# ewrfcas/LeftRefill

Hardware: AMD Instinct MI355X
Metric: 512x1024 stitched images/sec @ 50 DDIM steps, cfg=2.5; per-UNet-step ms (higher is better)
Workload: dtype f16; 1 GPU; configs[1]: 1-ref inpainting, 512x1024 canvas (latent 64x128), B=4 per GPU (UNet batch 8 under CFG), 50 DDIM steps, cfg=2.5, eta=1.0, fp16; global_batch=4, per_gpu_batch=4, ddim_steps=50, parallelism=dp1 (sample-sharded, no data-path collective), ranks=1

## Files before the change

include/leftrefill_hip.h:

```cpp
#ifndef LEFTREFILL_HIP_H
#define LEFTREFILL_HIP_H

#include <stdint.h>

#ifdef __cplusplus
extern "C" {
#endif

#define LR_E_ARG (-1)
#define LR_E_ALIGN (-2)
#define LR_E_UNSUPPORTED (-3)

typedef void* lr_stream_t;
typedef uint16_t lr_half;
#define LR_DTYPE_F16 0
#define LR_DTYPE_BF16 1
#define LR_PIPE_DEFAULT 0
#define LR_PIPE_W8_DEEP 4
#define LR_PIPE_HALO 8
#define LR_UP_PHASE 3

int lr_abi_version(void);

int lr_nchw_f32_to_nhwc_f16(const float* x1, int C1, const float* x2, int C2, lr_half* y, int Cpad, int N, int H,
// ... 53 lines not shown
} lr_gemm_args;
int lr_gemm_gn_group_chunks(const lr_gemm_args* args);
int lr_gemm_gn_rows(const lr_gemm_args* args);
int lr_gemm_plan(const lr_gemm_args* args, int32_t* plan);
int lr_gemm_stats_parts(const lr_gemm_args* args);
int64_t lr_gemm_workspace_bytes(const lr_gemm_args* args);
int lr_gemm_conv_f16(const lr_gemm_args* args, lr_stream_t s);
int lr_gemm_splitk_timeouts(void);

int lr_attention_f16(const lr_half* q, int ldq, const lr_half* k, int ldk, const lr_half* v, int ldv, lr_half* o,
                     int ldo, int B, int heads, int Nq, int Nkv, float scale, lr_stream_t s);

int lr_attention_causal_f16(const lr_half* q, int ldq, const lr_half* k, int ldk, const lr_half* v, int ldv, lr_half* o,
                            int ldo, int B, int heads, int N, float scale, lr_stream_t s);
int lr_attention_vt_f16(const lr_half* q, int ldq, const lr_half* k, int ldk, const lr_half* vt, int ld_vt, lr_half* o,
                        int ldo, int B, int heads, int Nq, int Nkv, float scale, lr_stream_t s);
int lr_transpose_v_f16(const lr_half* v, int ldv, lr_half* vt, int ld_vt, int B, int heads, int Nkv, lr_stream_t s);

typedef struct lr_xattn_args {
  const lr_half* x; lr_half* out;
  const lr_half* wq; const float* bq;
  const lr_half* k; int32_t ldk;
  const lr_half* vt;
  const lr_half* wo; const float* bo;
  float* stats_out;
  int32_t M, HW, C, heads, Lc;
  float ln_eps, scale;
  const lr_half* pre_a; const lr_half* pre_w; const float* pre_b;
} lr_xattn_args;
int lr_xattn_block_f16(const lr_xattn_args* args, lr_stream_t s);
int lr_xattn_pack_vt_f16(const lr_half* v, int ldv, lr_half* vt, int B, int heads, int Lc, lr_stream_t s);

typedef struct lr_stin_args {
  const lr_half* x; const lr_half* wp; const float* bp; const lr_half* wqkv; const float* bqkv;
  lr_half* x1; lr_half* qkv;
  int32_t M, C, NQ, ld_qkv;
  float ln_eps;
  const float* gn_part; const float* gn_gamma; const float* gn_beta;
  int32_t gn_chunks, gn_hw;
  float gn_eps;
} lr_stin_args;
int lr_stin_block_f16(const lr_stin_args* args, lr_stream_t s);

typedef struct lr_rowlin_args {
  const lr_half* x; const lr_half* w; const float* bias; lr_half* out;
  int32_t M, C, N, ld_out, geglu;
  float ln_eps;
  int32_t ln;
  const float* gn_part; const float* gn_gamma; const float* gn_beta;
  int32_t gn_chunks, gn_hw;
  float gn_eps;
} lr_rowlin_args;
int lr_rowlin_f16(const lr_rowlin_args* args, lr_stream_t s);

typedef struct lr_ffn_args {
  const lr_half* x; lr_half* out;
  const lr_half* w1; const float* b1;
  const lr_half* w2; const float* b2;
  float* stats_out;
  int32_t M, C, H;
  float ln_eps;
  const lr_half* post_w; const float* post_b; const lr_half* post_resid; float* gn_stats_out;
  float* gn_group_out; int32_t gn_hw;
} lr_ffn_args;
int lr_ffn_block_f16(const lr_ffn_args* args, lr_stream_t s);

int lr_softmax_rows_f16(const lr_half* s, lr_half* p, int M, int N, float scale, lr_stream_t st);

int lr_mv_gather(const lr_half* x, lr_half* seq, int b, int v, int s, int C, lr_stream_t st);
typedef struct lr_row_copy_job {
  const void* src; int64_t src_pitch, src_off;
  void* dst; int64_t dst_pitch, dst_off;
  int32_t row_bytes, n_rows;
  const int32_t* src_idx; const int32_t* dst_idx;
} lr_row_copy_job;
int lr_row_copy(const lr_row_copy_job* jobs, int n_jobs, lr_stream_t s);
int lr_mv_scatter(const lr_half* seq, lr_half* x, int b, int v, int s, int C, lr_stream_t st);

int lr_ddim_cfg_step(const float* x, const void* eps, int eps_is_f32, const float* noise, float* x_prev,
                     float* pred_x0, int64_t numel, float cfg_scale, float a_t, float a_prev, float sigma_t,
                     float sqrt_one_minus_at, lr_stream_t s);

int lr_plms_cfg_step(const float* x, const void* eps, int eps_is_f32, const float* const* hist, int n_hist, const float* weights,
                     float divisor, float* e_out, float* x_prev, float* pred_x0, int64_t numel, float cfg_scale, float a_t,
                     float a_prev, float sqrt_one_minus_at, lr_stream_t s);

int lr_dpmpp_cfg_step(const float* x, const void* eps, int eps_is_f32, const float* x0_prev, float* x0_out, float* x_next,
                      int64_t numel, float cfg_scale, float sigma_s, float alpha_s, float ratio, float c, float c_half,
                      float inv_r0, lr_stream_t s);

int lr_ddim_inv_cfg_step(const float* x, const void* eps, int eps_is_f32, float* x_next, int64_t numel, float cfg_scale,
                         float c1, float c2, lr_stream_t s);

int lr_ddim_cfg3_step(const float* x, const void* eps, int eps_is_f32, const float* noise, float* x_prev, float* pred_x0,
                      int64_t numel, float cfg_scale, float cond_weight, float one_minus_cond_weight, float a_t, float a_prev,
                      float sigma_t, float sqrt_one_minus_at, lr_stream_t s);

int lr_ddpm_step(const float* x, const void* eps, int eps_is_f32, const float* noise, const float* known_x0,
                 const float* known_noise, const float* mask, int64_t mask_chw, int64_t mask_hw, int clip_denoised, float* x_prev,
                 float* x0_out, int64_t numel, float sqrt_recip_ac, float sqrt_recipm1_ac, float coef1, float coef2, float sigma,
                 float sqrt_ac, float sqrt_one_minus_ac, lr_stream_t s);

#define LR_Q_SAMPLE_MAX_B 32
int lr_ddim_q_sample(const float* x0, const float* noise, float* out, int B, int64_t per_sample, const float* sa,
                     const float* s1ma, lr_stream_t s);

// ... 280 lines not shown
```

leftrefill_amd/_lib.py:

```python
import ctypes
import os

HERE = os.path.dirname(os.path.abspath(__file__))
LIB_PATH = os.environ.get("LEFTREFILL_LIB_PATH") or os.path.join(HERE, "lib", "libleftrefill_hip.so")
ABI_VERSION = 30

c_void_p, c_int, c_float, c_int64 = ctypes.c_void_p, ctypes.c_int, ctypes.c_float, ctypes.c_int64


class GemmArgs(ctypes.Structure):
    _fields_ = [
        ("p1", c_void_p), ("C1", ctypes.c_int32),
        ("p2", c_void_p), ("C2", ctypes.c_int32),
        ("B", ctypes.c_int32), ("H", ctypes.c_int32), ("W", ctypes.c_int32),
        ("Hs", ctypes.c_int32), ("Ws", ctypes.c_int32),
        ("taps", ctypes.c_int32), ("stride", ctypes.c_int32), ("up", ctypes.c_int32),
        ("asym", ctypes.c_int32),
        ("wt", c_void_p), ("N", ctypes.c_int32),
        ("bias", c_void_p),
        ("rowvec", c_void_p), ("ld_rowvec", ctypes.c_int32),
        ("resid", c_void_p), ("ld_resid", ctypes.c_int32),
        ("out", c_void_p), ("ld_out", ctypes.c_int32),
        ("geglu", ctypes.c_int32),
        ("tile_n", ctypes.c_int32),
# ... 147 lines not shown
                                    c_float, c_void_p],
    "lr_attention_causal_bwd_f16": [ctypes.POINTER(AttnBwdArgs), c_void_p],
    "lr_gelu_fwd_f16": [c_void_p, c_void_p, c_int64, c_void_p],
    "lr_gelu_bwd_f16": [c_void_p, c_void_p, c_void_p, c_int64, c_void_p],
    "lr_transpose_v_f16": [c_void_p, c_int, c_void_p, c_int, c_int, c_int, c_int, c_void_p],
    "lr_xattn_block_f16": [ctypes.POINTER(XattnArgs), c_void_p],
    "lr_xattn_pack_vt_f16": [c_void_p, c_int, c_void_p, c_int, c_int, c_int, c_void_p],
    "lr_ffn_block_f16": [ctypes.POINTER(FfnArgs), c_void_p],
    "lr_stin_block_f16": [ctypes.POINTER(StinArgs), c_void_p],
    "lr_rowlin_f16": [ctypes.POINTER(RowlinArgs), c_void_p],
    "lr_mv_gather": [c_void_p, c_void_p, c_int, c_int, c_int, c_int, c_void_p],
    "lr_row_copy": [c_void_p, c_int, c_void_p],
    "lr_gemm_splitk_timeouts": [],
    "lr_mv_scatter": [c_void_p, c_void_p, c_int, c_int, c_int, c_int, c_void_p],
    "lr_ddim_cfg_step": [c_void_p, c_void_p, c_int, c_void_p, c_void_p, c_void_p, c_int64, c_float, c_float, c_float,
                         c_float, c_float, c_void_p],
    "lr_timestep_embedding_f32": [c_void_p, c_int, c_int, c_void_p, c_void_p],
    "lr_plms_cfg_step": [c_void_p, c_void_p, c_int, c_void_p, c_int, c_void_p, c_float, c_void_p, c_void_p, c_void_p, c_int64,
                         c_float, c_float, c_float, c_float, c_void_p],
    "lr_dpmpp_cfg_step": [c_void_p, c_void_p, c_int, c_void_p, c_void_p, c_void_p, c_int64, c_float, c_float, c_float, c_float,
                          c_float, c_float, c_float, c_void_p],
    "lr_ddim_inv_cfg_step": [c_void_p, c_void_p, c_int, c_void_p, c_int64, c_float, c_float, c_float, c_void_p],
    "lr_ddim_cfg3_step": [c_void_p, c_void_p, c_int, c_void_p, c_void_p, c_void_p, c_int64, c_float, c_float, c_float, c_float,
                          c_float, c_float, c_float, c_void_p],
    "lr_ddpm_step": [c_void_p, c_void_p, c_int, c_void_p, c_void_p, c_void_p, c_void_p, c_int64, c_int64, c_int, c_void_p, c_void_p,
                     c_int64, c_float, c_float, c_float, c_float, c_float, c_float, c_float, c_void_p],
    "lr_ddim_q_sample": [c_void_p, c_void_p, c_void_p, c_int, c_int64, c_void_p, c_void_p, c_void_p],
    "lr_eval_metrics": [c_void_p, c_int, c_void_p, c_void_p, c_int, c_int, c_int, c_int, c_int, c_int, c_void_p, c_void_p, c_void_p,
                        c_void_p],
    "lr_amp_adamw_step": [c_void_p, c_int, c_void_p, c_int, c_void_p, c_void_p, c_int, c_float, c_float, c_int,
                          ctypes.POINTER(c_int), c_void_p],
    "lr_lpips_workspace_bytes": [c_int, c_int, c_int, c_int],
    "lr_lpips_alex": [ctypes.POINTER(LpipsArgs), c_void_p],
    "lr_batch_prep": [c_void_p, c_int64, c_void_p, c_void_p, c_int, c_int, c_int, c_int, c_void_p, c_void_p, c_void_p, c_void_p],
    "lr_nvs_prep": [c_void_p, c_int64, c_void_p, c_void_p, c_int, c_int, c_void_p, c_void_p, c_void_p, c_void_p],
    "lr_pil_resize": [c_void_p, c_int64, c_void_p, c_void_p, c_int64, c_void_p, c_int64, c_void_p, c_int64, c_void_p, c_void_p, c_int,
                      c_void_p],
    "lr_refill_canvas": [c_void_p, c_void_p, c_void_p, c_int, c_int, c_int, c_int, c_int, c_int, c_void_p, c_void_p, c_void_p, c_void_p],
    "lr_image_grid": [ctypes.POINTER(GridSource), c_int, c_int, c_int, c_int, c_int, c_void_p, c_int, c_void_p],
    "lr_token_drift": [c_void_p, c_void_p, c_int, c_int, c_void_p, c_void_p],
    "lr_attention_probe_f16": [c_void_p, c_int, c_void_p, c_int, c_void_p, c_int, c_int, c_void_p, c_int, c_int, c_int, c_int, c_float,
                               c_float, c_float, c_void_p],
    "lr_lora_down_f16": [c_void_p, c_int, c_void_p, c_int, c_void_p, c_int, c_int, c_int, c_int, c_float, c_void_p],
    "lr_lora_up_f16": [c_void_p, c_int, c_void_p, c_int, c_void_p, c_int, c_int, c_int, c_int, c_int, c_void_p],
    "lr_lora_wgrad_workspace_bytes": [c_int, c_int, c_int],
    "lr_lora_wgrad_f16": [c_void_p, c_int, c_void_p, c_int, c_void_p, c_int, c_int, c_int, c_int, c_float, c_void_p, c_int64, c_void_p],
    "lr_lora_merge_f32": [c_void_p, c_void_p, c_void_p, c_void_p, c_int, c_int, c_int, c_float, c_void_p],
    "lr_lora_down_drop_f16": [c_void_p, c_int, c_void_p, c_int, c_void_p, c_int, c_int, c_int, c_int, c_float, ctypes.POINTER(LoraDrop),
                              c_void_p],
    "lr_lora_up_drop_f16": [c_void_p, c_int, c_void_p, c_int, c_void_p, c_int, c_int, c_int, c_int, c_int, ctypes.POINTER(LoraDrop),
                            c_void_p],
    "lr_lora_wgrad_drop_f16": [c_void_p, c_int, c_void_p, c_int, c_void_p, c_int, c_int, c_int, c_int, c_float, c_void_p, c_int64,
                               ctypes.POINTER(LoraDrop), c_void_p],
}
INT64_RETURNS = ("lr_gemm_workspace_bytes", "lr_lpips_workspace_bytes", "lr_lora_wgrad_workspace_bytes")

BF16_TWINS = ["lr_groupnorm_stats", "lr_groupnorm_apply", "lr_groupnorm_apply_n", "lr_layernorm", "lr_layernorm_bwd",
              "lr_groupnorm_bwd", "lr_layernorm_bwd_res", "lr_groupnorm_bwd_res", "lr_nchw_f32_to_nhwc_f16", "lr_nhwc_f16_to_nchw", "lr_timestep_embedding", "lr_linear_small_m",
              "lr_mv_gather", "lr_mv_scatter", "lr_ddim_cfg_step", "lr_timestep_embedding_f32", "lr_plms_cfg_step",
              "lr_dpmpp_cfg_step", "lr_ddim_inv_cfg_step", "lr_ddim_cfg3_step", "lr_ddpm_step", "lr_geglu_fwd", "lr_geglu_bwd", "lr_sumpool2x2",
              "lr_mv_gather_bwd", "lr_mv_scatter_bwd", "lr_attention_f16", "lr_attention_causal_f16", "lr_attention_lse_f16",
              "lr_attention_vt_f16", "lr_transpose_v_f16", "lr_attention_bwd_f16", "lr_xattn_block_f16",
              "lr_xattn_pack_vt_f16", "lr_ffn_block_f16", "lr_stin_block_f16", "lr_rowlin_f16", "lr_gn_conv_out_f16",
              "lr_attention_causal_lse_f16", "lr_attention_causal_bwd_f16", "lr_gelu_fwd_f16", "lr_gelu_bwd_f16",
              "lr_attention_probe_f16", "lr_lora_down_f16", "lr_lora_up_f16", "lr_lora_wgrad_f16",
              "lr_lora_down_drop_f16", "lr_lora_up_drop_f16", "lr_lora_wgrad_drop_f16"]


def twin(name):
    return (name[:-4] if name.endswith("_f16") else name) + "_bf16"


for _n in BF16_TWINS:
    SIGNATURES[twin(_n)] = SIGNATURES[_n]

_FOLD_SIG = [c_void_p, c_int, c_int, c_int, c_int, c_void_p, c_void_p, c_float, c_void_p, c_void_p, c_int, c_void_p, c_void_p, c_void_p]
DEV_SIGNATURES = {"lr_dev_set": [ctypes.c_char_p, c_int], "lr_dev_unset": [ctypes.c_char_p],
                  "lr_gn_fold_weights_f16": _FOLD_SIG, "lr_gn_fold_weights_bf16": _FOLD_SIG}

_lib = None


def fn(lib, name, dtype):
    import torch
    if dtype == torch.bfloat16:
        return getattr(lib, twin(name))
    assert dtype == torch.float16, dtype
    return getattr(lib, name)


def load():
    global _lib
    if _lib is not None:
        return _lib
    import torch
    if not os.path.exists(LIB_PATH):
        raise RuntimeError(
            f"{LIB_PATH} not found: build it with `python -m leftrefill_amd.build` (hipcc --offload-arch=gfx950). "
            "leftrefill_amd has no fallback path.")
    lib = ctypes.CDLL(LIB_PATH)
    for name, argtypes in SIGNATURES.items():
        fn = getattr(lib, name)
        fn.argtypes = argtypes
        fn.restype = c_int64 if name in INT64_RETURNS else c_int
    v = lib.lr_abi_version()
    if v != ABI_VERSION:
# ... 32 lines not shown
```

leftrefill_amd/csrc/rowlin.hip:

```cpp
#include "chain_common.h"

#define RL_ROWS 128
#define RL_THREADS 512
#define RL_SLOT 40960
#ifndef RL_DMA_AUX
#define RL_DMA_AUX 0
#endif
#ifndef RL_DEPTH
#define RL_DEPTH 1
#endif
#ifndef RL_W4_DEFAULT
#define RL_W4_DEFAULT 0
#endif
#define RL_MAX_SLICE 2560

struct RowlinParams {
  const void* x; const void* w; const float* bias; void* out;
  int M, N, ld_out, ny, np;
  float eps;
  const float* gn_part; const float* gn_gamma; const float* gn_beta; int gn_chunks, gn_hw; float gn_eps;
};

template <typename T, int C, bool GEGLU, bool LN, bool GN = false>
__global__ __launch_bounds__(RL_THREADS) void rowlin_kernel(const RowlinParams P) {
#if defined(__HIP_DEVICE_COMPILE__)
  constexpr int KL = C / 64;
  constexpr int NKS = C / 320;
  constexpr int RS = C == 320 ? 2 : 1;
  constexpr int UPR = GEGLU ? 1 : 2;
  constexpr int NU = RS * UPR;
  constexpr int S = NU;
  extern __shared__ __attribute__((aligned(16))) char smem[];
  float* par = reinterpret_cast<float*>(smem + 3 * RL_SLOT);

  const int t = threadIdx.x, lane = t & 63;
  const int w = __builtin_amdgcn_readfirstlane(t >> 6);
  const int fr = lane & 15, fq = lane >> 4;
  const int odd = fq & 1, ch8 = (fq >> 1) * 8;
  const int rb = blockIdx.x / P.ny, y = blockIdx.x - rb * P.ny;
  const int m_w0 = rb * (RL_ROWS * RS) + w * 16 * RS;
  const int np = P.np;
  const int g_base = y * np;
  const int j0 = rb % np;

  vec8<T> xf[RS][KL][2];
#pragma unroll
  for (int rs = 0; rs < RS; ++rs) {
    const T* xrow = reinterpret_cast<const T*>(P.x) + (size_t)(m_w0 + 16 * rs + fr) * C + 8 * fq;
#pragma unroll
    for (int t5 = 0; t5 < KL; ++t5)
#pragma unroll
      for (int u = 0; u < 2; ++u) xf[rs][t5][u] = *reinterpret_cast<const vec8<T>*>(xrow + 64 * t5 + 32 * u);
  }
  for (int i = t; i < np * 16; i += RL_THREADS)
    *reinterpret_cast<f32x4*>(par + 4 * i) = *reinterpret_cast<const f32x4*>(P.bias + (size_t)g_base * 64 + 4 * i);

  const __amdgpu_buffer_rsrc_t rsW = uniform_rsrc(P.w, (size_t)P.N * C * 2);
  const unsigned OOB = 0x80000000u;
  const int lrow = w * 8 + (lane >> 3);
  const int lchunk = (lane & 7) ^ ((lrow >> 1) & 7);
  const unsigned vrow = (unsigned)((lrow * C + lchunk * 8) * 2);
  auto issue = [&](int slot, int g, int kh, int i, bool live) __attribute__((always_inline)) {
    __builtin_amdgcn_raw_ptr_buffer_load_lds(rsW, (lptr_t)(smem + slot * RL_SLOT + (i * 64 + w * 8) * 128), 16, live ? vrow : OOB,
                                             (g * 64 * C + 320 * kh + i * 64) * 2, 0, RL_DMA_AUX);
  };
  auto piece_of = [&](int j) -> int { const int q = j0 + j; return g_base + (q < np ? q : q - np); };
  {
    const int g0 = piece_of(0);
#pragma unroll
    for (int i = 0; i < 5; ++i) issue(0, g0, 0, i, true);
#pragma unroll
    for (int i = 0; i < 5; ++i) {
      if constexpr (NKS == 1) issue(1, np > 1 ? piece_of(1) : g0, 0, i, np > 1); else issue(1, g0, 1, i, true);
    }
  }

  if constexpr (GN) {
    float* tabA = par + RL_MAX_SLICE;
    float* tabB = tabA + C;
    xa_gn_tables(P.gn_part, P.gn_chunks, (rb * (RL_ROWS * RS)) / P.gn_hw, P.gn_hw, C, P.gn_gamma, P.gn_beta, P.gn_eps, tabA, tabB, tabB + C, t, RL_THREADS);
#pragma unroll
    for (int rs = 0; rs < RS; ++rs)
#pragma unroll
      for (int t5 = 0; t5 < KL; ++t5)
#pragma unroll
        for (int u = 0; u < 2; ++u) {
          const int c0 = 64 * t5 + 32 * u + 8 * fq;
          const f32x4 a0 = *reinterpret_cast<const f32x4*>(tabA + c0), a1 = *reinterpret_cast<const f32x4*>(tabA + c0 + 4);
          const f32x4 b0 = *reinterpret_cast<const f32x4*>(tabB + c0), b1 = *reinterpret_cast<const f32x4*>(tabB + c0 + 4);
#pragma unroll
          for (int i = 0; i < 4; ++i) {
            xf[rs][t5][u][i] = (T)fmaf((float)xf[rs][t5][u][i], a0[i], b0[i]);
            xf[rs][t5][u][4 + i] = (T)fmaf((float)xf[rs][t5][u][4 + i], a1[i], b1[i]);
          }
        }
  }
  if constexpr (LN) {
#pragma unroll
    for (int rs = 0; rs < RS; ++rs) {
      __builtin_amdgcn_sched_barrier(0);
      float sm = 0.f;
#pragma unroll
      for (int t5 = 0; t5 < KL; ++t5)
#pragma unroll
        for (int u = 0; u < 2; ++u)
#pragma unroll
          for (int i = 0; i < 8; ++i) sm += (float)xf[rs][t5][u][i];
      const float mean = xa_row4_sum(sm) * (1.0f / C);
#pragma unroll
      for (int t5 = 0; t5 < KL; ++t5)
#pragma unroll
        for (int u = 0; u < 2; ++u) asm volatile("" : "+v"(xf[rs][t5][u]));
      float q2 = 0.f;
#pragma unroll
      for (int t5 = 0; t5 < KL; ++t5)
#pragma unroll
        for (int u = 0; u < 2; ++u)
#pragma unroll
          for (int i = 0; i < 8; ++i) { const float d = (float)xf[rs][t5][u][i] - mean; q2 = fmaf(d, d, q2); }
      const float rstd = rsqrtf(xa_row4_sum(q2) * (1.0f / C) + P.eps);
      const float nmr = -mean * rstd;
#pragma unroll
      for (int t5 = 0; t5 < KL; ++t5)
#pragma unroll
        for (int u = 0; u < 2; ++u) asm volatile("" : "+v"(xf[rs][t5][u]));
#pragma unroll
      for (int t5 = 0; t5 < KL; ++t5)
#pragma unroll
        for (int u = 0; u < 2; ++u)
#pragma unroll
          for (int i = 0; i < 8; ++i) xf[rs][t5][u][i] = (T)fmaf((float)xf[rs][t5][u][i], rstd, nmr);
    }
  }

  const int sw = (fr >> 1) & 7;
  auto frag = [&](const char* base, int row, int chunk) -> vec8<T> {
    return *reinterpret_cast<const vec8<T>*>(base + row * 128 + ((chunk ^ sw) << 4));
  };
  const f32x4 z4 = {0.f, 0.f, 0.f, 0.f};
  T* outp = reinterpret_cast<T*>(P.out);
  auto emit_unit = [&](const f32x4 (&accs)[RS][4], int lp, int g, int uu) __attribute__((always_inline)) {
    const int rs = uu / UPR, u = uu % UPR;
    const f32x4 (&acc)[4] = accs[rs];
    const float* b = par + lp * 64 + 4 * fq;
    f32x4 a, c;
    int col;
    if constexpr (GEGLU) {
      const f32x4 u0 = acc[0] + *reinterpret_cast<const f32x4*>(b), g0 = acc[1] + *reinterpret_cast<const f32x4*>(b + 16);
      const f32x4 u1 = acc[2] + *reinterpret_cast<const f32x4*>(b + 32), g1 = acc[3] + *reinterpret_cast<const f32x4*>(b + 48);
      const f32x2_t e0 = lr_gelu_erf2((f32x2_t){g0[0], g0[1]}), e1 = lr_gelu_erf2((f32x2_t){g0[2], g0[3]});
      const f32x2_t e2 = lr_gelu_erf2((f32x2_t){g1[0], g1[1]}), e3 = lr_gelu_erf2((f32x2_t){g1[2], g1[3]});
      a = (f32x4){u0[0] * e0[0], u0[1] * e0[1], u0[2] * e1[0], u0[3] * e1[1]};
      c = (f32x4){u1[0] * e2[0], u1[1] * e2[1], u1[2] * e3[0], u1[3] * e3[1]};
      col = g * 32 + odd * 16 + ch8;
    } else {
      a = acc[2 * u] + *reinterpret_cast<const f32x4*>(b + (2 * u) * 16);
      c = acc[2 * u + 1] + *reinterpret_cast<const f32x4*>(b + (2 * u + 1) * 16);
      col = g * 64 + (2 * u + odd) * 16 + ch8;
    }
    xa_swap_rows16(a, c);
    const float v[8] = {a[0], a[1], a[2], a[3], c[0], c[1], c[2], c[3]};
    const uint4 pk = lr_pack8<T>(v);
#ifdef RL_DBG_NOSTORE
    if (pk.x == 0x12345678u && pk.y == 0x9abcdef0u)
#endif
    *reinterpret_cast<uint4*>(outp + (size_t)(m_w0 + 16 * rs + fr) * P.ld_out + col) = pk;
  };

#define RL_FENCE() __builtin_amdgcn_sched_barrier(0)
#ifdef RL_DBG_NODMA
#define RL_DBG_DMA(X)
#else
#define RL_DBG_DMA(X) X
#endif
#ifdef RL_DBG_NOMFMA
#define RL_DBG_MFMA(X) acc[rs][jd][0] += (float)fa[ks % (RL_DEPTH + 1)][jd][0];
#else
#define RL_DBG_MFMA(X) X
#endif

#define RL_STEP(KH, NB, EMIT)                                                                                                      \
  {                                                                                                                                \
    { const int nb_ = (NB); if (nb_ == 2) xa_wait_vmcnt<5 + 2 * S>(); else if (nb_ == 1) xa_wait_vmcnt<5 + S>(); else xa_wait_vmcnt<5>(); } \
    asm volatile("s_waitcnt lgkmcnt(0)" ::: "memory");                                                                             \
    __builtin_amdgcn_s_barrier();                                                                                                  \
    const char* Ws = smem + slot * RL_SLOT;                                                                                        \
    const int slot2 = slot == 0 ? 2 : slot - 1;                                                                \
    constexpr int po_ = ((KH) + 2) / NKS, kh2_ = ((KH) + 2) % NKS;                                                                 \
    const int g2_ = po_ == 0 ? g : po_ == 1 ? g_next : g_next2;                                                                    \
    const bool live2_ = po_ == 0 ? true : po_ == 1 ? more : more2;                                                                 \
    vec8<T> fa[RL_DEPTH + 1][4];                                                                                                   \
    auto rd = [&](int ks, vec8<T> (&f)[4]) __attribute__((always_inline)) {                                                        \
      _Pragma("unroll") for (int jd = 0; jd < 4; ++jd) f[jd] = frag(Ws + (ks >> 1) * 64 * 128, jd * 16 + fr, 4 * (ks & 1) + fq);   \
    };                                                                                                                             \
    _Pragma("unroll") for (int d_ = 0; d_ < RL_DEPTH; ++d_) rd(d_, fa[d_]);                                                        \
    _Pragma("unroll") for (int ks = 0; ks < 10; ++ks) {                                                                            \
      if (ks + RL_DEPTH < 10) rd(ks + RL_DEPTH, fa[(ks + RL_DEPTH) % (RL_DEPTH + 1)]);                                             \
      RL_FENCE();                                                                                                                  \
      _Pragma("unroll") for (int jd = 0; jd < 4; ++jd)                                                                             \
        _Pragma("unroll") for (int rs = 0; rs < RS; ++rs)                                                                          \
          RL_DBG_MFMA(acc[rs][jd] = lr_mfma16(fa[ks % (RL_DEPTH + 1)][jd], xf[rs][5 * (KH) + (ks >> 1)][ks & 1], ((KH) == 0 && ks == 0) ? z4 : acc[rs][jd]);) \
      RL_DBG_DMA(if (ks < 5) issue(slot2, g2_, kh2_, ks, live2_);)                                                                 \
      { constexpr int st_ = NU == 4 ? 1 : 2;                                                                                       \
        if (ks >= 5 && (ks - 5) % st_ == 0 && (ks - 5) / st_ < NU) { const int u = (ks - 5) / st_; EMIT; } }                       \
      RL_FENCE();                                                                                                                  \
    }                                                                                                                              \
    slot = slot == 2 ? 0 : slot + 1;                                                                                               \
  }

  f32x4 acc[RS][4], prev[RS][4];
  int slot = 0, g_prev = 0;
#pragma unroll 1
  for (int j = 0; j < np; ++j) {
    const int g = piece_of(j);
    const bool more = j + 1 < np, more2 = j + 2 < np;
    const int g_next = more ? piece_of(j + 1) : g, g_next2 = more2 ? piece_of(j + 2) : g;
    if constexpr (NKS == 1) {
      RL_STEP(0, (j >= 3) + (j >= 2), { if (j > 0) emit_unit(prev, g_prev - g_base, g_prev, u); });
    } else if constexpr (NKS == 2) {
      RL_STEP(0, j >= 2, { if (j > 0) emit_unit(prev, g_prev - g_base, g_prev, u); });
      RL_STEP(1, j >= 1, { });
    } else {
      RL_STEP(0, 0, { if (j > 0) emit_unit(prev, g_prev - g_base, g_prev, u); });
      RL_STEP(1, j >= 1, { });
      RL_STEP(2, j >= 1, { });
      RL_STEP(3, 0, { });
    }
#pragma unroll
    for (int rs = 0; rs < RS; ++rs)
#pragma unroll
      for (int jd = 0; jd < 4; ++jd) prev[rs][jd] = acc[rs][jd];
    g_prev = g;
  }
#pragma unroll
  for (int u = 0; u < NU; ++u) emit_unit(prev, g_prev - g_base, g_prev, u);
  xa_wait_vmcnt<0>();
#undef RL_STEP
#undef RL_FENCE
#endif
}

#ifdef LR_DEV_VARIANTS
#define R4_THREADS 256
#define R4_SLOT 20480
#define R4_ROWS 128
template <typename T, bool GEGLU, bool LN, bool GN>
__global__ __launch_bounds__(R4_THREADS, 2) void rowlin4_kernel(const RowlinParams P) {
#if defined(__HIP_DEVICE_COMPILE__)
  constexpr int C = 640, KL = 10, RS = 2;
  constexpr int S = RS;
  extern __shared__ __attribute__((aligned(16))) char smem[];
  float* par = reinterpret_cast<float*>(smem + 3 * R4_SLOT);

  const int t = threadIdx.x, lane = t & 63;
  const int w = __builtin_amdgcn_readfirstlane(t >> 6);
  const int fr = lane & 15, fq = lane >> 4;
  const int odd = fq & 1, ch8 = (fq >> 1) * 8;
  const int rb = blockIdx.x / P.ny, y = blockIdx.x - rb * P.ny;
  const int m_w0 = rb * R4_ROWS + w * 32;
  const int np = P.np;
  const int g_base = y * np;
  const int j0 = rb % np;

  vec8<T> xf[RS][KL][2];
#pragma unroll
  for (int rs = 0; rs < RS; ++rs) {
    const T* xrow = reinterpret_cast<const T*>(P.x) + (size_t)(m_w0 + 16 * rs + fr) * C + 8 * fq;
#pragma unroll
    for (int t5 = 0; t5 < KL; ++t5)
#pragma unroll
      for (int u = 0; u < 2; ++u) xf[rs][t5][u] = *reinterpret_cast<const vec8<T>*>(xrow + 64 * t5 + 32 * u);
  }
  for (int i = t; i < np * 8; i += R4_THREADS)
    *reinterpret_cast<f32x4*>(par + 4 * i) = *reinterpret_cast<const f32x4*>(P.bias + (size_t)g_base * 32 + 4 * i);

  const __amdgpu_buffer_rsrc_t rsW = uniform_rsrc(P.w, (size_t)P.N * C * 2);
  const unsigned OOB = 0x80000000u;
  const int lrow = w * 8 + (lane >> 3);
  const int lchunk = (lane & 7) ^ ((lrow >> 1) & 7);
  const unsigned vrow = (unsigned)((lrow * C + lchunk * 8) * 2);
  auto issue = [&](int slot, int g, int kh, int i, bool live) __attribute__((always_inline)) {
    __builtin_amdgcn_raw_ptr_buffer_load_lds(rsW, (lptr_t)(smem + slot * R4_SLOT + (i * 32 + w * 8) * 128), 16, live ? vrow : OOB,
                                             (g * 32 * C + 320 * kh + i * 64) * 2, 0, RL_DMA_AUX);
  };
  auto piece_of = [&](int j) -> int { const int q = j0 + j; return g_base + (q < np ? q : q - np); };
  {
    const int g0 = piece_of(0);
#pragma unroll
// ... 117 lines not shown
#pragma unroll 1
  for (int j = 0; j < np; ++j) {
    const int g = piece_of(j);
    const bool more = j + 1 < np;
    const int g_next = more ? piece_of(j + 1) : g;
    R4_STEP(0, j >= 2, { if (j > 0) emit_unit(prev, g_prev - g_base, g_prev, u); });
    R4_STEP(1, j >= 1, { });
#pragma unroll
    for (int rs = 0; rs < RS; ++rs)
#pragma unroll
      for (int jd = 0; jd < 2; ++jd) prev[rs][jd] = acc[rs][jd];
    g_prev = g;
  }
#pragma unroll
  for (int u = 0; u < RS; ++u) emit_unit(prev, g_prev - g_base, g_prev, u);
  xa_wait_vmcnt<0>();
#undef R4_STEP
#undef R4_FENCE
#endif
}

template <typename T, bool GEGLU, bool LN, bool GN>
static int rowlin4_launch(const RowlinParams& P, hipStream_t st) {
  const size_t smem = 3 * R4_SLOT + (size_t)(RL_MAX_SLICE + (GN ? 2 * 640 + 64 : 0)) * sizeof(float);
  static unsigned long long attr_done = 0;
  return lr_launch_dyn(rowlin4_kernel<T, GEGLU, LN, GN>, &attr_done, dim3((P.M / R4_ROWS) * P.ny), dim3(R4_THREADS), smem, st, P);
}

static int rowlin4_ny(int M, int N) {
  const int rbs = M / R4_ROWS, pieces = N / 32;
  int want = 512 / (rbs > 0 ? rbs : 1);
  if (want < 1) want = 1;
  int ny = 0;
  for (int d = 1; d <= pieces && d <= want; ++d)
    if (pieces % d == 0 && pieces / d >= 3 && pieces / d * 32 <= RL_MAX_SLICE) ny = d;
  return ny;
}
#endif

static int rowlin_ny(int M, int N, int rows) {
  const int rbs = M / rows, pieces = N / 64;
  int want = 256 / (rbs > 0 ? rbs : 1);
  if (want < 1) want = 1;
  int ny = 1;
  for (int d = 1; d <= pieces && d <= want; ++d)
    if (pieces % d == 0 && pieces / d * 64 <= RL_MAX_SLICE) ny = d;
  while (pieces / ny * 64 > RL_MAX_SLICE && ny < pieces) {
    ++ny;
    while (ny < pieces && pieces % ny) ++ny;
  }
  return ny;
}

template <typename T, int C, bool GEGLU, bool LN, bool GN = false>
static int rowlin_launch(const RowlinParams& P, hipStream_t st) {
  const size_t smem = 3 * RL_SLOT + (size_t)(RL_MAX_SLICE + (GN ? 2 * C + 64 : 0)) * sizeof(float);
  static unsigned long long attr_done = 0;
  return lr_launch_dyn(rowlin_kernel<T, C, GEGLU, LN, GN>, &attr_done, dim3((P.M / (C == 320 ? 2 * RL_ROWS : RL_ROWS)) * P.ny), dim3(RL_THREADS), smem, st, P);
}

template <typename T>
static int rowlin_t(const lr_rowlin_args* a, lr_stream_t s) {
  if (!a || !a->x || !a->w || !a->bias || !a->out) return LR_E_ARG;
  if (a->M <= 0 || a->N <= 0 || (a->geglu != 0 && a->geglu != 1) || (a->ln != 0 && a->ln != 1)) return LR_E_ARG;
  const int rows = a->C == 320 ? 2 * RL_ROWS : RL_ROWS;
#ifdef LR_DEV_VARIANTS
  if ((a->C != 320 && a->C != 640 && a->C != 1280) || a->M % rows || a->N % 64) return LR_E_UNSUPPORTED;
#else
  if (a->C != 640 || a->M % rows || a->N % 64) return LR_E_UNSUPPORTED;
#endif
  if (a->geglu && !a->ln) return LR_E_UNSUPPORTED;
  const int n_out = a->geglu ? a->N / 2 : a->N;
  if (a->ld_out < n_out || a->ld_out % 8) return LR_E_ALIGN;
  if (((uintptr_t)a->x | (uintptr_t)a->w | (uintptr_t)a->bias | (uintptr_t)a->out) & 15) return LR_E_ALIGN;
  if ((int64_t)a->N * a->C * 2 >= ((int64_t)1 << 31)) return LR_E_UNSUPPORTED;
  RowlinParams P;
  P.x = a->x; P.w = a->w; P.bias = a->bias; P.out = a->out;
  P.M = a->M; P.N = a->N; P.ld_out = a->ld_out; P.eps = a->ln_eps;
  P.ny = rowlin_ny(a->M, a->N, rows);
  P.np = a->N / 64 / P.ny;
  if (P.np * 64 > RL_MAX_SLICE) return LR_E_UNSUPPORTED;
  hipStream_t st = (hipStream_t)s;
  const bool gn = a->gn_part != nullptr;
  if (gn) {
    if (a->C != 640 || a->ln || a->geglu) return LR_E_UNSUPPORTED;
    if (!a->gn_gamma || !a->gn_beta || a->gn_chunks <= 0 || a->gn_hw <= 0) return LR_E_ARG;
    if (a->gn_hw % rows || a->M % a->gn_hw) return LR_E_UNSUPPORTED;
    if (((uintptr_t)a->gn_part & 7) || (((uintptr_t)a->gn_gamma | (uintptr_t)a->gn_beta) & 3)) return LR_E_ALIGN;
  }
  P.gn_part = a->gn_part; P.gn_gamma = a->gn_gamma; P.gn_beta = a->gn_beta; P.gn_chunks = a->gn_chunks; P.gn_hw = a->gn_hw; P.gn_eps = a->gn_eps;
#ifdef LR_DEV_VARIANTS
  if (a->C == 640 && LR_DEV("LR_ROWLIN_W4", RL_W4_DEFAULT)) {
    const int ny4 = rowlin4_ny(a->M, a->N);
    if (ny4 > 0) {
      P.ny = ny4;
      P.np = a->N / 32 / ny4;
      if (gn) return rowlin4_launch<T, false, false, true>(P, st);
      if (a->geglu) return rowlin4_launch<T, true, true, false>(P, st);
      return a->ln ? rowlin4_launch<T, false, true, false>(P, st) : rowlin4_launch<T, false, false, false>(P, st);
    }
  }
#endif
  if (gn) return rowlin_launch<T, 640, false, false, true>(P, st);
#ifdef LR_DEV_VARIANTS
  if (a->C == 320) {
    if (a->geglu) return rowlin_launch<T, 320, true, true>(P, st);
    return LR_E_UNSUPPORTED;
  }
#endif
  if (a->C == 640) {
    if (a->geglu) return rowlin_launch<T, 640, true, true>(P, st);
    return a->ln ? rowlin_launch<T, 640, false, true>(P, st) : rowlin_launch<T, 640, false, false>(P, st);
  }
#ifdef LR_DEV_VARIANTS
  if (a->geglu) return rowlin_launch<T, 1280, true, true>(P, st);
  return a->ln ? rowlin_launch<T, 1280, false, true>(P, st) : rowlin_launch<T, 1280, false, false>(P, st);
#else
  return LR_E_UNSUPPORTED;
#endif
}

extern "C" int lr_rowlin_f16(const lr_rowlin_args* a, lr_stream_t s) { return rowlin_t<f16>(a, s); }
extern "C" int lr_rowlin_bf16(const lr_rowlin_args* a, lr_stream_t s) { return rowlin_t<bf16>(a, s); }
```

leftrefill_amd/ops.py:

```python
import ctypes
import os

import torch

from . import _lib
from ._lib import FfnArgs, GemmArgs, RowlinArgs, StinArgs, XattnArgs

GN_CHUNKS = 256
GN_GROUPS = os.environ.get("LEFTREFILL_GN_GROUPS", "1") != "0"

AUTOTUNE = os.environ.get("LEFTREFILL_AUTOTUNE", "0") == "1"
TILE_CANDIDATES = ((128, 64, 0), (128, 128, 0), (128, 160, 0), (128, 128, 4), (128, 160, 4), (256, 128, 0), (256, 160, 0),
                   (256, 256, 0), (256, 320, 0), (256, 160, 8), (256, 320, 8))
TILE_TABLE_PATH = os.environ.get("LEFTREFILL_TILE_TABLE_PATH",
                                 os.path.join(os.path.dirname(os.path.abspath(__file__)), "tile_table.json"))
_tile_cache = None
PLAN_LOG = os.environ.get("LEFTREFILL_PLAN_LOG", "0") == "1"
SPLITK_MODE = int(os.environ.get("LEFTREFILL_SPLITK_MODE", "0"))
_untabulated = set()
TABLE_HITS, TABLE_MISSES = set(), set()
PLAN_TRIAL = None
LAUNCH_HOOK = None


# ... 545 lines not shown
        assert pa_.shape == (M, C) and pw_.dtype == x.dtype and pw_.is_contiguous() and pw_.shape == (C, C)
        assert pb_.dtype == torch.float32 and pb_.numel() == C
        a.pre_a, a.pre_w, a.pre_b = _p(pa_), _p(pw_), _p(pb_)
    _lib.check(_fn(lib, "lr_xattn_block_f16", x.dtype)(a, _stream()), "xattn_block")
    return (out, stats) if want_stats else out


STIN_C, STIN_ROWS = 320, 256


def stin_ok(M, C, NQ):
    return C == STIN_C and M % STIN_ROWS == 0 and NQ > 0 and NQ % 192 == 0 and NQ <= 4096


def stin_block(x, wp, bp, wqkv, bqkv, *, eps, out=None, qkv_out=None, gn=None):
    lib = _lib.load()
    _chk16(x, "x")
    M, C = x.shape
    NQ = wqkv.shape[0]
    assert stin_ok(M, C, NQ), (M, C, NQ)
    assert wp.dtype == x.dtype and wp.is_contiguous() and wp.shape == (C, C) and wqkv.dtype == x.dtype and wqkv.is_contiguous() and wqkv.shape == (NQ, C)
    assert bp.dtype == torch.float32 and bp.numel() == C and bqkv.dtype == torch.float32 and bqkv.numel() == NQ
    x1 = torch.empty_like(x) if out is None else out
    qkv = torch.empty(M, NQ, device=x.device, dtype=x.dtype) if qkv_out is None else qkv_out
    assert x1.shape == x.shape and x1.is_contiguous() and qkv.shape == (M, NQ) and qkv.stride(1) == 1 and qkv.dtype == x.dtype
    a = StinArgs()
    a.x, a.wp, a.bp, a.wqkv, a.bqkv, a.x1, a.qkv = _p(x), _p(wp), _p(bp), _p(wqkv), _p(bqkv), _p(x1), _p(qkv)
    a.M, a.C, a.NQ, a.ld_qkv, a.ln_eps = M, C, NQ, qkv.stride(0), float(eps)
    a.gn_part = a.gn_gamma = a.gn_beta = 0
    a.gn_chunks = a.gn_hw = 0
    a.gn_eps = 0.0
    if gn is not None:
        gp, chunks, hw, gamma, beta, geps = gn
        assert gp.dtype == torch.float32 and gp.is_contiguous() and gp.shape == (M // hw, chunks, 32, 2) and hw % STIN_ROWS == 0
        assert gamma.dtype == torch.float32 and beta.dtype == torch.float32 and gamma.numel() == C and beta.numel() == C
        a.gn_part, a.gn_gamma, a.gn_beta, a.gn_chunks, a.gn_hw, a.gn_eps = _p(gp), _p(gamma), _p(beta), int(chunks), int(hw), float(geps)
    _lib.check(_fn(lib, "lr_stin_block_f16", x.dtype)(a, _stream()), "stin_block")
    return x1, qkv


ROWLIN_ROWS = 128
ROWLIN_WIDTHS = {"qkv": (640,), "q": (), "in": (640,), "geglu": (640,)}
FFN_SPLIT = os.environ.get("LEFTREFILL_FFN_SPLIT", "0") != "0"
ROWLIN_MIN_ROWS = 2048
ROWLIN = os.environ.get("LEFTREFILL_ROWLIN", "1") != "0"


def rowlin_ok(M, C, N, kind="qkv"):
    if kind == "geglu" and C == 320:
        return ROWLIN and FFN_SPLIT and _lib.dev_variants() and M % (2 * ROWLIN_ROWS) == 0 and M >= 8 * ROWLIN_MIN_ROWS and N > 0 and N % 64 == 0 and N <= 2560
    return ROWLIN and C in ROWLIN_WIDTHS.get(kind, ()) and M % ROWLIN_ROWS == 0 and M >= ROWLIN_MIN_ROWS and N > 0 and N % 64 == 0


def rowlin(x, w, bias, *, eps=1e-5, geglu=False, ln=True, out=None, gn=None):
    lib = _lib.load()
    _chk16(x, "x")
    M, C = x.shape
    N = w.shape[0]
    assert C in (320, 640, 1280) and M % (ROWLIN_ROWS * (2 if C == 320 else 1)) == 0 and N % 64 == 0, (M, C, N)
    assert w.dtype == x.dtype and w.is_contiguous() and w.shape == (N, C) and bias.dtype == torch.float32 and bias.numel() == N
    n_out = N // 2 if geglu else N
    if out is None:
        out = torch.empty(M, n_out, device=x.device, dtype=x.dtype)
    assert out.shape == (M, n_out) and out.stride(1) == 1 and out.dtype == x.dtype
    a = RowlinArgs()
    a.x, a.w, a.bias, a.out = _p(x), _p(w), _p(bias), _p(out)
    a.M, a.C, a.N, a.ld_out, a.geglu, a.ln_eps, a.ln = M, C, N, out.stride(0), int(bool(geglu)), float(eps), int(bool(ln))
    a.gn_part = a.gn_gamma = a.gn_beta = 0
    a.gn_chunks = a.gn_hw = 0
    a.gn_eps = 0.0
    if gn is not None:
        gp, chunks, hw, gamma, beta, geps = gn
        assert not ln and not geglu and gp.dtype == torch.float32 and gp.is_contiguous() and gp.shape == (M // hw, chunks, 32, 2) and hw % ROWLIN_ROWS == 0
        assert gamma.dtype == torch.float32 and beta.dtype == torch.float32 and gamma.numel() == C and beta.numel() == C
        a.gn_part, a.gn_gamma, a.gn_beta, a.gn_chunks, a.gn_hw, a.gn_eps = _p(gp), _p(gamma), _p(beta), int(chunks), int(hw), float(geps)
    _lib.check(_fn(lib, "lr_rowlin_f16", x.dtype)(a, _stream()), "rowlin")
    return out


FFN_C, FFN_ROWS, FFN_MAX_H = 320, 128, 2048


def ffn_ok(M, C, H):
    return C == FFN_C and M % FFN_ROWS == 0 and H % 64 == 0 and 0 < H <= FFN_MAX_H


def ffn_block(x, w1, b1, w2, b2, *, eps, want_stats=False, out=None, post=None, want_gn_stats=False, gn_hw=0):
    lib = _lib.load()
    _chk16(x, "x")
    M, C = x.shape
    H = w2.shape[0] * 64
    assert ffn_ok(M, C, H), (M, C, H)
    assert w1.dtype == x.dtype and w1.is_contiguous() and w1.shape == (2 * H, C)
    assert w2.dtype == x.dtype and w2.is_contiguous() and w2.shape == (H // 64, C, 64)
    assert b1.dtype == torch.float32 and b1.numel() == 2 * H and b2.dtype == torch.float32 and b2.numel() == C
    if out is None:
        out = torch.empty_like(x)
    assert out.shape == x.shape and out.dtype == x.dtype and out.is_contiguous() and out.device == x.device
    stats = torch.empty(M, 2, 2, device=x.device, dtype=torch.float32) if want_stats else None
    a = FfnArgs()
    a.x, a.out, a.w1, a.b1, a.w2, a.b2, a.stats_out = _p(x), _p(out), _p(w1), _p(b1), _p(w2), _p(b2), _p(stats)
    a.M, a.C, a.H, a.ln_eps = M, C, H, float(eps)
    a.post_w = a.post_b = a.post_resid = a.gn_stats_out = 0
    a.gn_group_out, a.gn_hw = 0, 0
    gstats = None
    if post is not None:
# ... 451 lines not shown
```

Before: 4.877 images/s.

## Add 256-row rowlin tiles for C=640 GEGLU with half-width weight pieces

Adds an RS template parameter so the C=640 row-linear kernel can process two 16-row sets per wave (256 rows per block), with a new HALF path that streams 32-column weight halves and interleaves emission across two half-steps. A plan function picks 256-row tiles by default for the GEGLU form (forms mask 2), which halves weight traffic per output row and the number of blocks. It also exposes the plan through a C and Python API. The cost is higher register pressure, a more complex pipelining and wait schedule, and fewer blocks, which may reduce occupancy or parallelism.

Result: no change. 4.887 images/s (median of 6 runs) (+0.2%).

```diff
diff --git a/include/leftrefill_hip.h b/include/leftrefill_hip.h
--- a/include/leftrefill_hip.h
+++ b/include/leftrefill_hip.h
@@ -129,6 +129,7 @@
   float gn_eps;
 } lr_rowlin_args;
 int lr_rowlin_f16(const lr_rowlin_args* args, lr_stream_t s);
+int lr_rowlin_plan(int32_t M, int32_t C, int32_t N, int32_t form, int32_t gn_hw, int32_t* rows, int32_t* ny);
 
 typedef struct lr_ffn_args {
   const lr_half* x; lr_half* out;
diff --git a/leftrefill_amd/_lib.py b/leftrefill_amd/_lib.py
--- a/leftrefill_amd/_lib.py
+++ b/leftrefill_amd/_lib.py
@@ -223,6 +223,7 @@
                             c_void_p],
     "lr_lora_wgrad_drop_f16": [c_void_p, c_int, c_void_p, c_int, c_void_p, c_int, c_int, c_int, c_int, c_float, c_void_p, c_int64,
                                ctypes.POINTER(LoraDrop), c_void_p],
+    "lr_rowlin_plan": [c_int, c_int, c_int, c_int, c_int, ctypes.POINTER(ctypes.c_int32), ctypes.POINTER(ctypes.c_int32)],
 }
 INT64_RETURNS = ("lr_gemm_workspace_bytes", "lr_lpips_workspace_bytes", "lr_lora_wgrad_workspace_bytes")
 
diff --git a/leftrefill_amd/csrc/rowlin.hip b/leftrefill_amd/csrc/rowlin.hip
--- a/leftrefill_amd/csrc/rowlin.hip
+++ b/leftrefill_amd/csrc/rowlin.hip
@@ -21,12 +21,13 @@
   const float* gn_part; const float* gn_gamma; const float* gn_beta; int gn_chunks, gn_hw; float gn_eps;
 };
 
-template <typename T, int C, bool GEGLU, bool LN, bool GN = false>
+template <typename T, int C, int RS, bool GEGLU, bool LN, bool GN = false>
 __global__ __launch_bounds__(RL_THREADS) void rowlin_kernel(const RowlinParams P) {
 #if defined(__HIP_DEVICE_COMPILE__)
+  static_assert(RS == 1 || RS == 2, "one or two 16-row sets per wave");
   constexpr int KL = C / 64;
   constexpr int NKS = C / 320;
-  constexpr int RS = C == 320 ? 2 : 1;
+  constexpr bool HALF = C == 640 && RS == 2;
   constexpr int UPR = GEGLU ? 1 : 2;
   constexpr int NU = RS * UPR;
   constexpr int S = NU;
@@ -57,21 +58,22 @@
 
   const __amdgpu_buffer_rsrc_t rsW = uniform_rsrc(P.w, (size_t)P.N * C * 2);
   const unsigned OOB = 0x80000000u;
-  const int lrow = w * 8 + (lane >> 3);
+  const int lrow = HALF ? (w & 3) * 8 + (lane >> 3) : w * 8 + (lane >> 3);
   const int lchunk = (lane & 7) ^ ((lrow >> 1) & 7);
-  const unsigned vrow = (unsigned)((lrow * C + lchunk * 8) * 2);
+  const unsigned vrow = (unsigned)((lrow * C + (HALF ? (w >> 2) * 64 : 0) + lchunk * 8) * 2);
   auto issue = [&](int slot, int g, int kh, int i, bool live) __attribute__((always_inline)) {
     __builtin_amdgcn_raw_ptr_buffer_load_lds(rsW, (lptr_t)(smem + slot * RL_SLOT + (i * 64 + w * 8) * 128), 16, live ? vrow : OOB,
-                                             (g * 64 * C + 320 * kh + i * 64) * 2, 0, RL_DMA_AUX);
+                                             HALF ? (g * 32 * C + i * 128) * 2 : (g * 64 * C + 320 * kh + i * 64) * 2, 0, RL_DMA_AUX);
   };
   auto piece_of = [&](int j) -> int { const int q = j0 + j; return g_base + (q < np ? q : q - np); };
   {
     const int g0 = piece_of(0);
 #pragma unroll
-    for (int i = 0; i < 5; ++i) issue(0, g0, 0, i, true);
+    for (int i = 0; i < 5; ++i) issue(0, HALF ? 2 * g0 : g0, 0, i, true);
 #pragma unroll
     for (int i = 0; i < 5; ++i) {
-      if constexpr (NKS == 1) issue(1, np > 1 ? piece_of(1) : g0, 0, i, np > 1); else issue(1, g0, 1, i, true);
+      if constexpr (HALF) issue(1, 2 * g0 + 1, 0, i, true);
+      else if constexpr (NKS == 1) issue(1, np > 1 ? piece_of(1) : g0, 0, i, np > 1); else issue(1, g0, 1, i, true);
     }
   }
 
@@ -93,6 +95,7 @@
             xf[rs][t5][u][i] = (T)fmaf((float)xf[rs][t5][u][i], a0[i], b0[i]);
             xf[rs][t5][u][4 + i] = (T)fmaf((float)xf[rs][t5][u][4 + i], a1[i], b1[i]);
           }
+          if constexpr (HALF) asm volatile("" : "+v"(xf[rs][t5][u]));
         }
   }
   if constexpr (LN) {
@@ -127,9 +130,11 @@
 #pragma unroll
       for (int t5 = 0; t5 < KL; ++t5)
 #pragma unroll
-        for (int u = 0; u < 2; ++u)
+        for (int u = 0; u < 2; ++u) {
 #pragma unroll
           for (int i = 0; i < 8; ++i) xf[rs][t5][u][i] = (T)fmaf((float)xf[rs][t5][u][i], rstd, nmr);
+          if constexpr (HALF) asm volatile("" : "+v"(xf[rs][t5][u]));
+        }
     }
   }
 
@@ -208,6 +213,94 @@
     slot = slot == 2 ? 0 : slot + 1;                                                                                               \
   }
 
+  if constexpr (HALF) {
+  f32x4 acc[RS][2], prev[RS][2], ga[GEGLU ? RS : 1];
+  auto emit_half = [&](const f32x4 (&accs)[RS][2], int lh, int gh, int rs, bool second) __attribute__((always_inline)) {
+    const f32x4 (&ac)[2] = accs[rs];
+    const float* b = par + lh * 32 + 4 * fq;
+    f32x4 a, c;
+    int col;
+    if constexpr (GEGLU) {
+      const f32x4 u0 = ac[0] + *reinterpret_cast<const f32x4*>(b), g0 = ac[1] + *reinterpret_cast<const f32x4*>(b + 16);
+      const f32x2_t e0 = lr_gelu_erf2((f32x2_t){g0[0], g0[1]}), e1 = lr_gelu_erf2((f32x2_t){g0[2], g0[3]});
+      const f32x4 v = (f32x4){u0[0] * e0[0], u0[1] * e0[1], u0[2] * e1[0], u0[3] * e1[1]};
+      if (!second) { ga[rs] = v; return; }
+      a = ga[rs];
+      c = v;
+      col = (gh >> 1) * 32 + odd * 16 + ch8;
+    } else {
+      a = ac[0] + *reinterpret_cast<const f32x4*>(b);
+      c = ac[1] + *reinterpret_cast<const f32x4*>(b + 16);
+      col = gh * 32 + odd * 16 + ch8;
+    }
+    xa_swap_rows16(a, c);
+    const float v8[8] = {a[0], a[1], a[2], a[3], c[0], c[1], c[2], c[3]};
+    const uint4 pk = lr_pack8<T>(v8);
+#ifdef RL_DBG_NOSTORE
+    if (pk.x == 0x12345678u && pk.y == 0x9abcdef0u)
+#endif
+    *reinterpret_cast<uint4*>(outp + (size_t)(m_w0 + 16 * rs + fr) * P.ld_out + col) = pk;
+  };
+#ifndef RL_H_DMA_EVERY
+#define RL_H_DMA_EVERY 1
+#endif
+#ifndef RL_H_DEPTH
+#define RL_H_DEPTH 1
+#endif
+#ifndef RL_H_EMIT0
+#define RL_H_EMIT0 6
+#endif
+static_assert(RL_H_EMIT0 > 4 * RL_H_DMA_EVERY && RL_H_EMIT0 + 6 < 20, "a step's stores follow its five LDS-DMA (the counted waits of RL_HSTEP)");
+#ifdef RL_DBG_NOMFMA
+#define RL_H_MFMA(X) acc[rs][jd][0] += (float)fa[ks % (RL_H_DEPTH + 1)][jd][0];
+#else
+#define RL_H_MFMA(X) X
+#endif
+#define RL_HSTEP(HF, NB, EMIT)                                                                                                     \
+  {                                                                                                                                \
+    { const int nb_ = (NB); if (nb_ == 2) xa_wait_vmcnt<5 + 2 * RS>(); else if (nb_ == 1) xa_wait_vmcnt<5 + RS>(); else xa_wait_vmcnt<5>(); } \
+    asm volatile("s_waitcnt lgkmcnt(0)" ::: "memory");                                                                             \
+    __builtin_amdgcn_s_barrier();                                                                                                  \
+    const char* Ws = smem + slot * RL_SLOT;                                                                                        \
+    const int slot2 = slot == 0 ? 2 : slot - 1;                                                                \
+    vec8<T> fa[RL_H_DEPTH + 1][2];                                                                                                 \
+    auto rd = [&](int ks, vec8<T> (&f)[2]) __attribute__((always_inline)) {                                                        \
+      _Pragma("unroll") for (int jd = 0; jd < 2; ++jd) f[jd] = frag(Ws + (ks >> 1) * 32 * 128, jd * 16 + fr, 4 * (ks & 1) + fq);   \
+    };                                                                                                                             \
+    _Pragma("unroll") for (int d_ = 0; d_ < RL_H_DEPTH; ++d_) rd(d_, fa[d_]);                                                      \
+    _Pragma("unroll") for (int ks = 0; ks < 20; ++ks) {                                                                            \
+      if (ks + RL_H_DEPTH < 20) rd(ks + RL_H_DEPTH, fa[(ks + RL_H_DEPTH) % (RL_H_DEPTH + 1)]);                                     \
+      RL_FENCE();                                                                                                                  \
+      _Pragma("unroll") for (int jd = 0; jd < 2; ++jd)                                                                             \
+        _Pragma("unroll") for (int rs = 0; rs < RS; ++rs)                                                                          \
+          RL_H_MFMA(acc[rs][jd] = lr_mfma16(fa[ks % (RL_H_DEPTH + 1)][jd], xf[rs][ks >> 1][ks & 1], ks == 0 ? z4 : acc[rs][jd]);)  \
+      RL_DBG_DMA(if (ks % RL_H_DMA_EVERY == 0 && ks / RL_H_DMA_EVERY < 5) issue(slot2, 2 * g_next + (HF), 0, ks / RL_H_DMA_EVERY, more);)\
+      if (ks == RL_H_EMIT0 || ks == RL_H_EMIT0 + 6) { const int u = (ks - RL_H_EMIT0) / 6; EMIT; }                                 \
+      RL_FENCE();                                                                                                                  \
+    }                                                                                                                              \
+    slot = slot == 2 ? 0 : slot + 1;                                                                                               \
+    _Pragma("unroll") for (int rs = 0; rs < RS; ++rs)                                                                              \
+      _Pragma("unroll") for (int jd = 0; jd < 2; ++jd) prev[rs][jd] = acc[rs][jd];                                                 \
+  }
+  int slot = 0, g_prev = 0;
+#pragma unroll 1
+  for (int j = 0; j < np; ++j) {
+    const int g = piece_of(j);
+    const bool more = j + 1 < np;
+    const int g_next = more ? piece_of(j + 1) : g;
+    if constexpr (GEGLU) {
+      RL_HSTEP(0, j >= 2, { if (j > 0) emit_half(prev, 2 * (g_prev - g_base) + 1, 2 * g_prev + 1, u, true); });
+      RL_HSTEP(1, j >= 1, { emit_half(prev, 2 * (g - g_base), 2 * g, u, false); });
+    } else {
+      RL_HSTEP(0, (j >= 1) + (j >= 2), { if (j > 0) emit_half(prev, 2 * (g_prev - g_base) + 1, 2 * g_prev + 1, u, true); });
+      RL_HSTEP(1, 2 * (j >= 1), { emit_half(prev, 2 * (g - g_base), 2 * g, u, false); });
+    }
+    g_prev = g;
+  }
+#pragma unroll
+  for (int rs = 0; rs < RS; ++rs) emit_half(prev, 2 * (g_prev - g_base) + 1, 2 * g_prev + 1, rs, true);
+#undef RL_HSTEP
+  } else {
   f32x4 acc[RS][4], prev[RS][4];
   int slot = 0, g_prev = 0;
 #pragma unroll 1
@@ -234,6 +327,7 @@
   }
 #pragma unroll
   for (int u = 0; u < NU; ++u) emit_unit(prev, g_prev - g_base, g_prev, u);
+  }
   xa_wait_vmcnt<0>();
 #undef RL_STEP
 #undef RL_FENCE
@@ -457,11 +551,26 @@
   return ny;
 }
 
-template <typename T, int C, bool GEGLU, bool LN, bool GN = false>
+struct RowlinPlan { int rows, ny; };
+#define RL_ROWS256_FORMS 2
+static RowlinPlan rowlin_plan(int M, int N, int C, int form, int gn_hw) {
+  RowlinPlan pl;
+  pl.rows = C == 320 ? 2 * RL_ROWS : RL_ROWS;
+  const int forms = LR_DEV("LR_ROWLIN_ROWS256", RL_ROWS256_FORMS);
+  if (C == 640 && ((forms >> form) & 1) && M % (2 * RL_ROWS) == 0 && (gn_hw <= 0 || gn_hw % (2 * RL_ROWS) == 0)) pl.rows = 2 * RL_ROWS;
+  pl.ny = rowlin_ny(M, N, pl.rows);
+#ifdef LR_DEV_VARIANTS
+  const int want = LR_DEV("LR_ROWLIN_NY256", 0);
+  if (pl.rows == 2 * RL_ROWS && C == 640 && want > 0 && (N / 64) % want == 0 && N / want <= RL_MAX_SLICE) pl.ny = want;
+#endif
+  return pl;
+}
+
+template <typename T, int C, int RS, bool GEGLU, bool LN, bool GN = false>
 static int rowlin_launch(const RowlinParams& P, hipStream_t st) {
   const size_t smem = 3 * RL_SLOT + (size_t)(RL_MAX_SLICE + (GN ? 2 * C + 64 : 0)) * sizeof(float);
   static unsigned long long attr_done = 0;
-  return lr_launch_dyn(rowlin_kernel<T, C, GEGLU, LN, GN>, &attr_done, dim3((P.M / (C == 320 ? 2 * RL_ROWS : RL_ROWS)) * P.ny), dim3(RL_THREADS), smem, st, P);
+  return lr_launch_dyn(rowlin_kernel<T, C, RS, GEGLU, LN, GN>, &attr_done, dim3((P.M / (RS * RL_ROWS)) * P.ny), dim3(RL_THREADS), smem, st, P);
 }
 
 template <typename T>
@@ -482,11 +591,13 @@
   RowlinParams P;
   P.x = a->x; P.w = a->w; P.bias = a->bias; P.out = a->out;
   P.M = a->M; P.N = a->N; P.ld_out = a->ld_out; P.eps = a->ln_eps;
-  P.ny = rowlin_ny(a->M, a->N, rows);
+  const bool gn = a->gn_part != nullptr;
+  const RowlinPlan pl = rowlin_plan(a->M, a->N, a->C, a->geglu ? 1 : a->ln ? 0 : 2, gn ? a->gn_hw : 0);
+  const bool two = a->C == 640 && pl.rows == 2 * RL_ROWS;
+  P.ny = pl.ny;
   P.np = a->N / 64 / P.ny;
   if (P.np * 64 > RL_MAX_SLICE) return LR_E_UNSUPPORTED;
   hipStream_t st = (hipStream_t)s;
-  const bool gn = a->gn_part != nullptr;
   if (gn) {
     if (a->C != 640 || a->ln || a->geglu) return LR_E_UNSUPPORTED;
     if (!a->gn_gamma || !a->gn_beta || a->gn_chunks <= 0 || a->gn_hw <= 0) return LR_E_ARG;
@@ -495,7 +606,7 @@
   }
   P.gn_part = a->gn_part; P.gn_gamma = a->gn_gamma; P.gn_beta = a->gn_beta; P.gn_chunks = a->gn_chunks; P.gn_hw = a->gn_hw; P.gn_eps = a->gn_eps;
 #ifdef LR_DEV_VARIANTS
-  if (a->C == 640 && LR_DEV("LR_ROWLIN_W4", RL_W4_DEFAULT)) {
+  if (a->C == 640 && !two && LR_DEV("LR_ROWLIN_W4", RL_W4_DEFAULT)) {
     const int ny4 = rowlin4_ny(a->M, a->N);
     if (ny4 > 0) {
       P.ny = ny4;
@@ -506,20 +617,27 @@
     }
   }
 #endif
-  if (gn) return rowlin_launch<T, 640, false, false, true>(P, st);
+#ifdef LR_DEV_VARIANTS
+  if (gn && two) return rowlin_launch<T, 640, 2, false, false, true>(P, st);
+#endif
+  if (gn) return rowlin_launch<T, 640, 1, false, false, true>(P, st);
 #ifdef LR_DEV_VARIANTS
   if (a->C == 320) {
-    if (a->geglu) return rowlin_launch<T, 320, true, true>(P, st);
+    if (a->geglu) return rowlin_launch<T, 320, 2, true, true>(P, st);
     return LR_E_UNSUPPORTED;
   }
 #endif
   if (a->C == 640) {
-    if (a->geglu) return rowlin_launch<T, 640, true, true>(P, st);
-    return a->ln ? rowlin_launch<T, 640, false, true>(P, st) : rowlin_launch<T, 640, false, false>(P, st);
-  }
-#ifdef LR_DEV_VARIANTS
-  if (a->geglu) return rowlin_launch<T, 1280, true, true>(P, st);
-  return a->ln ? rowlin_launch<T, 1280, false, true>(P, st) : rowlin_launch<T, 1280, false, false>(P, st);
+    if (two && a->geglu) return rowlin_launch<T, 640, 2, true, true>(P, st);
+#ifdef LR_DEV_VARIANTS
+    if (two) return a->ln ? rowlin_launch<T, 640, 2, false, true>(P, st) : rowlin_launch<T, 640, 2, false, false>(P, st);
+#endif
+    if (a->geglu) return rowlin_launch<T, 640, 1, true, true>(P, st);
+    return a->ln ? rowlin_launch<T, 640, 1, false, true>(P, st) : rowlin_launch<T, 640, 1, false, false>(P, st);
+  }
+#ifdef LR_DEV_VARIANTS
+  if (a->geglu) return rowlin_launch<T, 1280, 1, true, true>(P, st);
+  return a->ln ? rowlin_launch<T, 1280, 1, false, true>(P, st) : rowlin_launch<T, 1280, 1, false, false>(P, st);
 #else
   return LR_E_UNSUPPORTED;
 #endif
@@ -527,3 +645,15 @@
 
 extern "C" int lr_rowlin_f16(const lr_rowlin_args* a, lr_stream_t s) { return rowlin_t<f16>(a, s); }
 extern "C" int lr_rowlin_bf16(const lr_rowlin_args* a, lr_stream_t s) { return rowlin_t<bf16>(a, s); }
+
+extern "C" int lr_rowlin_plan(int M, int C, int N, int form, int gn_hw, int* rows, int* ny) {
+  if (!rows || !ny || M <= 0 || N <= 0 || form < 0 || form > 2 || gn_hw < 0) return LR_E_ARG;
+  if (C != 320 && C != 640 && C != 1280) return LR_E_UNSUPPORTED;
+  const int min_rows = C == 320 ? 2 * RL_ROWS : RL_ROWS;
+  if (M % min_rows || N % 64 || (gn_hw > 0 && (form != 2 || C != 640 || gn_hw % min_rows || M % gn_hw))) return LR_E_UNSUPPORTED;
+  const RowlinPlan pl = rowlin_plan(M, N, C, form, gn_hw);
+  if (N / 64 / pl.ny * 64 > RL_MAX_SLICE) return LR_E_UNSUPPORTED;
+  *rows = pl.rows;
+  *ny = pl.ny;
+  return 0;
+}
diff --git a/leftrefill_amd/ops.py b/leftrefill_amd/ops.py
--- a/leftrefill_amd/ops.py
+++ b/leftrefill_amd/ops.py
@@ -621,6 +621,14 @@
     return ROWLIN and C in ROWLIN_WIDTHS.get(kind, ()) and M % ROWLIN_ROWS == 0 and M >= ROWLIN_MIN_ROWS and N > 0 and N % 64 == 0
 
 
+def rowlin_plan(M, C, N, *, geglu=False, ln=True, gn_hw=0):
+    import ctypes
+    rows, ny = ctypes.c_int32(0), ctypes.c_int32(0)
+    form = 1 if geglu else 0 if ln else 2
+    _lib.check(_lib.load().lr_rowlin_plan(M, C, N, form, gn_hw, ctypes.byref(rows), ctypes.byref(ny)), "rowlin_plan")
+    return rows.value, ny.value
+
+
 def rowlin(x, w, bias, *, eps=1e-5, geglu=False, ln=True, out=None, gn=None):
     lib = _lib.load()
     _chk16(x, "x")
```
